# wenbowen123/iros20-6d-pose-tracking

Measured on AMD Instinct MI355X. Metric: RGB-D pair inferences/sec (176x176), higher is better.
Workload: dtype f32; 1 GPU; configs[1]: batch=64 synthetic 176x176 RGB-D pairs per GPU, random-init Se3TrackNet (reference state_dict surface), stage=full; pairs_per_gpu=64, global_batch=64, stage=full, frames=resident in HBM

## Files before the change

iros20-6d-pose-tracking_amd/csrc/wino64_fused.hip:

```cpp
#include "mfma_common.h"

namespace se3tn {

namespace {
constexpr int W64_TILES = 11;
constexpr int W64_PATCH = 2 * W64_TILES + 2;
constexpr int W64_PATCH_FLOATS = W64_PATCH * W64_PATCH * 32;
constexpr int W64_V_FLOATS = 128 * 32, W64_U_FLOATS = 64 * 32;
constexpr int W64_UBUFS = 2;
constexpr int W64_LDS_FLOATS = W64_PATCH_FLOATS + 2 * W64_V_FLOATS + W64_UBUFS * W64_U_FLOATS;
constexpr int W64_YLDS_FLOATS = W64_TILES * W64_TILES * (4 * 64 + 4);
constexpr size_t W64_LDS_BYTES = sizeof(float) * (W64_YLDS_FLOATS > W64_LDS_FLOATS ? W64_YLDS_FLOATS : W64_LDS_FLOATS);
}

__device__ __forceinline__ void bt_row(int i, int& r0, int& r1, float& c0, float& c1) {
  r0 = i == 0 ? 0 : 1;
  r1 = i == 3 ? 3 : 2;
  c0 = i == 2 ? -1.f : 1.f;
  c1 = (i == 0 || i == 3) ? -1.f : 1.f;
}
__device__ __forceinline__ void at_col(int i, float& a0, float& a1) {
  a0 = i == 3 ? 0.f : 1.f;
  a1 = i == 0 ? 0.f : (i == 1 ? 1.f : -1.f);
}

template <bool NA, bool NB>
__device__ __forceinline__ float add_pm(const float a, const float b) {
  float r;
  if constexpr (!NA && !NB) asm volatile("v_add_f32 %0, %1, %2" : "=v"(r) : "v"(a), "v"(b));
  else if constexpr (NA && !NB) asm volatile("v_sub_f32 %0, %2, %1" : "=v"(r) : "v"(a), "v"(b));
  else if constexpr (!NA && NB) asm volatile("v_sub_f32 %0, %1, %2" : "=v"(r) : "v"(a), "v"(b));
  else asm volatile("v_sub_f32 %0, -%1, %2" : "=v"(r) : "v"(a), "v"(b));
  return r;
}
template <int K>
__device__ __forceinline__ void acc_pm(float& y, const float m) {
  if constexpr (K > 0) asm volatile("v_add_f32 %0, %0, %1" : "+v"(y) : "v"(m));
  else if constexpr (K < 0) asm volatile("v_sub_f32 %0, %0, %1" : "+v"(y) : "v"(m));
}
struct W64Tab {
  static constexpr int bt_r0(int i) { return i == 0 ? 0 : 1; }
  static constexpr int bt_r1(int i) { return i == 3 ? 3 : 2; }
  static constexpr bool bt_n0(int i) { return i == 2; }
  static constexpr bool bt_n1(int i) { return i == 0 || i == 3; }
  static constexpr int at(int y, int i) { return y == 0 ? (i == 3 ? 0 : 1) : (i == 0 ? 0 : (i == 1 ? 1 : -1)); }
  static constexpr int off(int r, int s) { return (r * W64_PATCH + (s >> 1) + 12 * (s & 1)) * 32; }
};

struct Wino64Args {
  const float* in;
  const float* U;
  const float* bias;
  const float* res;
  float* out;
  int in_ld, res_ld, out_ld;
  int in_gs, res_gs, out_gs, bias_gs;
  long long u_gs;
  int n, groups;
};

template <int EPI>
__global__ __launch_bounds__(512) void wino64_fused_kernel(const Wino64Args a) {
  extern __shared__ __attribute__((aligned(16))) float smem[];
  float* patch = smem;
  float* Vb = smem + W64_PATCH_FLOATS;
  float* Ub = Vb + 2 * W64_V_FLOATS;

  const int tid = threadIdx.x, lane = tid & 63;
  const int wid = __builtin_amdgcn_readfirstlane(tid >> 6);
  const int rb = wid >> 1, cbk = wid & 1;
  const int l31 = lane & 31, hh = lane >> 5;

  const int g = blockIdx.x % a.groups, rest = blockIdx.x / a.groups;
  const int quad = rest & 3, img = rest >> 2;
  const int y0 = (quad >> 1) * 2 * W64_TILES, x0 = (quad & 1) * 2 * W64_TILES;
  constexpr int HP = 46;
  const float* __restrict__ in = a.in + (size_t)g * a.in_gs + ((size_t)(img * HP + y0) * HP + x0) * a.in_ld;
  const float* __restrict__ Ug = a.U + (size_t)g * a.u_gs;
  const unsigned lds0 = __builtin_amdgcn_readfirstlane(lds_addr_of(smem));

  const int ur = tid >> 3;
  const unsigned uvoff = (unsigned)(lds_rows::stage_src(ur, tid & 7) * 4);

#define W64_ISSUE_PATCH(CH)                                                                                     \
  {                                                                                                            \
    const float* pb_ = in + (CH) * 32;                                                                          \
    _Pragma("unroll") for (int j_ = 0; j_ < 9; ++j_) {                                \
      const int id_ = tid + 512 * j_, px_ = id_ >> 3, py_ = px_ / W64_PATCH, pxx_ = px_ - py_ * W64_PATCH;      \
      const int xs_ = pxx_ < 12 ? 2 * pxx_ : 2 * pxx_ - 23;           \
      glds16<0>(pb_, (unsigned)(((py_ * HP + xs_) * a.in_ld + (id_ & 7) * 4) * 4),                              \
                lds0 + (unsigned)((wid * 64 + 512 * j_) * 16));                                                 \
    }                                                                                                          \
  }
#define W64_ISSUE_U(CH, F, BUFI)                                                                                \
  glds16<0>(Ug + (size_t)((CH) * 16 + (F)) * W64_U_FLOATS, uvoff,                                              \
            lds0 + (unsigned)((W64_PATCH_FLOATS + 2 * W64_V_FLOATS + (BUFI) * W64_U_FLOATS + wid * 256) * 4));

  int tpix[2], tdst[2];
#pragma unroll
  for (int j = 0; j < 2; ++j) {
    const int tt = (tid + 512 * j) >> 3, tcb = tid & 7;
    const int ttr = tt < W64_TILES * W64_TILES ? tt : W64_TILES * W64_TILES - 1;
    const int tty = ttr / W64_TILES, ttx = ttr - tty * W64_TILES;
    tpix[j] = ((2 * tty) * W64_PATCH + ttx) * 32 + tcb * 4;
    tdst[j] = tt * 32 + lds_rows::slot_off(tt, tcb);
  }
#define W64_BT(F)                                                                                               \
  int r0_, r1_, s0_, s1_;                                                                                      \
  float cr0_, cr1_, cs0_, cs1_;                                                                                \
  bt_row((F) >> 2, r0_, r1_, cr0_, cr1_);                                                                      \
  bt_row((F) & 3, s0_, s1_, cs0_, cs1_);                                                                       \
  const int q0_ = (s0_ >> 1) + 12 * (s0_ & 1), q1_ = (s1_ >> 1) + 12 * (s1_ & 1);              \
  const int o00_ = (r0_ * W64_PATCH + q0_) * 32, o01_ = (r0_ * W64_PATCH + q1_) * 32;                          \
  const int o10_ = (r1_ * W64_PATCH + q0_) * 32, o11_ = (r1_ * W64_PATCH + q1_) * 32;                          \
  const float c00_ = cr0_ * cs0_, c01_ = cr0_ * cs1_, c10_ = cr1_ * cs0_, c11_ = cr1_ * cs1_;
#define W64_TR_LOAD(D)                                                                                          \
  _Pragma("unroll") for (int j_ = 0; j_ < 2; ++j_) {                                                            \
    D[j_][0] = *reinterpret_cast<const float4*>(patch + tpix[j_] + o00_);                                       \
    D[j_][1] = *reinterpret_cast<const float4*>(patch + tpix[j_] + o01_);                                       \
    D[j_][2] = *reinterpret_cast<const float4*>(patch + tpix[j_] + o10_);                                       \
    D[j_][3] = *reinterpret_cast<const float4*>(patch + tpix[j_] + o11_);                                       \
  }
#define W64_TR_STORE(D, VBUF)                                                                                   \
  _Pragma("unroll") for (int j_ = 0; j_ < 2; ++j_) {                                                            \
    float4 v_;                                                                                                 \
    v_.x = c00_ * D[j_][0].x + c01_ * D[j_][1].x + c10_ * D[j_][2].x + c11_ * D[j_][3].x;                       \
    v_.y = c00_ * D[j_][0].y + c01_ * D[j_][1].y + c10_ * D[j_][2].y + c11_ * D[j_][3].y;                       \
    v_.z = c00_ * D[j_][0].z + c01_ * D[j_][1].z + c10_ * D[j_][2].z + c11_ * D[j_][3].z;                       \
    v_.w = c00_ * D[j_][0].w + c01_ * D[j_][1].w + c10_ * D[j_][2].w + c11_ * D[j_][3].w;                       \
    *reinterpret_cast<float4*>(Vb + (VBUF) * W64_V_FLOATS + tdst[j_]) = v_;                                     \
  }
#define W64_TRANSFORM(F, VBUF)                                                                                  \
  {                                                                                                            \
    W64_BT(F)                                                                                                  \
    float4 d_[2][4];                                                                                           \
    W64_TR_LOAD(d_)                                                                                            \
    W64_TR_STORE(d_, VBUF)                                                                                     \
  }

  const lds_rows::LaneFrag fo = lds_rows::lane_frag(l31, hh);

  float Y[16][4];
#pragma unroll
  for (int e = 0; e < 16; ++e)
#pragma unroll
    for (int o = 0; o < 4; ++o) Y[e][o] = 0.f;

  W64_ISSUE_PATCH(0)
  W64_ISSUE_U(0, 0, 0)
  wait_dma_and_barrier();
  W64_TRANSFORM(0, 0)
  __syncthreads();

  f32x16 accA, accB;
#pragma unroll
  for (int e = 0; e < 16; ++e) accB[e] = 0.f;
  const f32x16 zero16 = {0.f, 0.f, 0.f, 0.f, 0.f, 0.f, 0.f, 0.f, 0.f, 0.f, 0.f, 0.f, 0.f, 0.f, 0.f, 0.f};
#define W64_FOLD(PREV, F)                                                                                       \
  {                                                                                                            \
    float ay0_, ay1_, ax0_, ax1_;                                                                              \
    at_col((F) >> 2, ay0_, ay1_);                                                                              \
    at_col((F) & 3, ax0_, ax1_);                                                                               \
    const float k00_ = ay0_ * ax0_, k01_ = ay0_ * ax1_, k10_ = ay1_ * ax0_, k11_ = ay1_ * ax1_;                \
    _Pragma("unroll") for (int e_ = 0; e_ < 16; ++e_) {                                                        \
      const float m_ = PREV[e_];                                                                               \
      Y[e_][0] += k00_ * m_; Y[e_][1] += k01_ * m_; Y[e_][2] += k10_ * m_; Y[e_][3] += k11_ * m_;              \
    }                                                                                                          \
  }
#define W64_MFMA(ACC)                                                                                        \
  ACC = q_ == 0 ? __builtin_amdgcn_mfma_f32_32x32x2f32(wv_[0], pv_[0], zero16, 0, 0, 0)                         \
                : __builtin_amdgcn_mfma_f32_32x32x2f32(wv_[q_], pv_[q_], ACC, 0, 0, 0);
#define W64_STEP(F, ACC, PREV)                                                                                  \
  {                                                                                                            \
    constexpr int f_ = (F), buf = f_ & 1, fn_ = (f_ + 1) & 15, fp_ = (f_ + 15) & 15;                            \
    const bool last_ = ch == 1 && f_ == 15;                                                                    \
    if (!last_) W64_ISSUE_U(f_ == 15 ? 1 : ch, fn_, buf ^ 1)                                                    \
    if (f_ == 15 && ch == 0) W64_ISSUE_PATCH(1)  \
    {                                                                                                          \
      const float* pP = Vb + buf * W64_V_FLOATS + (rb * 32 + l31) * 32;                                        \
      const float* pW = Ub + buf * W64_U_FLOATS + (cbk * 32 + l31) * 32;                                       \
      float pv_[16], wv_[16];                                                                                  \
      float d_[2][4][4], v_[2][4];                                       \
      *reinterpret_cast<float4*>(pv_ + 0) = *reinterpret_cast<const float4*>(pP + fo.o0);                         \
      *reinterpret_cast<float4*>(wv_ + 0) = *reinterpret_cast<const float4*>(pW + fo.o0);                         \
      *reinterpret_cast<float4*>(pv_ + 4) = *reinterpret_cast<const float4*>(pP + fo.o1);                         \
      *reinterpret_cast<float4*>(wv_ + 4) = *reinterpret_cast<const float4*>(pW + fo.o1);                         \
      *reinterpret_cast<float4*>(pv_ + 8) = *reinterpret_cast<const float4*>(pP + fo.o2);                         \
      *reinterpret_cast<float4*>(wv_ + 8) = *reinterpret_cast<const float4*>(pW + fo.o2);                         \
      *reinterpret_cast<float4*>(pv_ + 12) = *reinterpret_cast<const float4*>(pP + fo.o3);                        \
      *reinterpret_cast<float4*>(wv_ + 12) = *reinterpret_cast<const float4*>(pW + fo.o3);                        \
                              \
       \
      constexpr int i_ = fn_ >> 2, j_ = fn_ & 3;                                                               \
      constexpr int oo_[4] = {W64Tab::off(W64Tab::bt_r0(i_), W64Tab::bt_r0(j_)), W64Tab::off(W64Tab::bt_r0(i_), W64Tab::bt_r1(j_)), \
                              W64Tab::off(W64Tab::bt_r1(i_), W64Tab::bt_r0(j_)), W64Tab::off(W64Tab::bt_r1(i_), W64Tab::bt_r1(j_))}; \
      constexpr bool nn_[4] = {W64Tab::bt_n0(i_) != W64Tab::bt_n0(j_), W64Tab::bt_n0(i_) != W64Tab::bt_n1(j_),  \
                               W64Tab::bt_n1(i_) != W64Tab::bt_n0(j_), W64Tab::bt_n1(i_) != W64Tab::bt_n1(j_)}; \
      _Pragma("unroll") for (int t_ = 0; t_ < 2; ++t_)                                                          \
        _Pragma("unroll") for (int w_ = 0; w_ < 4; ++w_)                                                        \
          *reinterpret_cast<float4*>(d_[t_][w_]) = *reinterpret_cast<const float4*>(patch + tpix[t_] + oo_[w_]); \
      constexpr int pi_ = fp_ >> 2, pj_ = fp_ & 3;    \
      __builtin_amdgcn_sched_barrier(0);                                                                       \
      _Pragma("unroll") for (int q_ = 0; q_ < 16; ++q_) {                                                       \
        W64_MFMA(ACC)                                                                                          \
        __builtin_amdgcn_sched_barrier(0);                                                                     \
        if (q_ < 8) {                             \
          _Pragma("unroll") for (int e_ = 2 * q_; e_ < 2 * q_ + 2; ++e_) {                                      \
            const float m_ = PREV[e_];                                                                         \
            acc_pm<W64Tab::at(0, pi_) * W64Tab::at(0, pj_)>(Y[e_][0], m_);                                     \
            acc_pm<W64Tab::at(0, pi_) * W64Tab::at(1, pj_)>(Y[e_][1], m_);                                     \
            acc_pm<W64Tab::at(1, pi_) * W64Tab::at(0, pj_)>(Y[e_][2], m_);                                     \
            acc_pm<W64Tab::at(1, pi_) * W64Tab::at(1, pj_)>(Y[e_][3], m_);                                     \
          }                                                                                                    \
        } else {               \
          const int t_ = (q_ - 8) >> 2, x_ = (q_ - 8) & 3;                                                     \
          v_[t_][x_] = add_pm<false, false>(add_pm<nn_[0], nn_[1]>(d_[t_][0][x_], d_[t_][1][x_]),              \
                                            add_pm<nn_[2], nn_[3]>(d_[t_][2][x_], d_[t_][3][x_]));             \
        }                                                                                                      \
        __builtin_amdgcn_sched_barrier(0);                                                                     \
      }                                                                                                        \
      *reinterpret_cast<float4*>(Vb + (buf ^ 1) * W64_V_FLOATS + tdst[0]) = *reinterpret_cast<float4*>(v_[0]); \
      *reinterpret_cast<float4*>(Vb + (buf ^ 1) * W64_V_FLOATS + tdst[1]) = *reinterpret_cast<float4*>(v_[1]); \
    }                                                                                                          \
    if (!last_) wait_dma_and_barrier();                                                                        \
    if (f_ == 15 && ch == 0) {  \
      W64_TRANSFORM(0, 0)                                                                                      \
      __syncthreads();                                                                                         \
    }                                                                                                          \
  }
  for (int ch = 0; ch < 2; ++ch) {
    W64_STEP(0, accA, accB) W64_STEP(1, accB, accA) W64_STEP(2, accA, accB) W64_STEP(3, accB, accA)
    W64_STEP(4, accA, accB) W64_STEP(5, accB, accA) W64_STEP(6, accA, accB) W64_STEP(7, accB, accA)
    W64_STEP(8, accA, accB) W64_STEP(9, accB, accA) W64_STEP(10, accA, accB) W64_STEP(11, accB, accA)
    W64_STEP(12, accA, accB) W64_STEP(13, accB, accA) W64_STEP(14, accA, accB) W64_STEP(15, accB, accA)
  }
  W64_FOLD(accB, 15)
#undef W64_STEP
#undef W64_MFMA
#undef W64_FOLD
#undef W64_ISSUE_PATCH
#undef W64_ISSUE_U
#undef W64_TRANSFORM
#undef W64_TR_LOAD
#undef W64_TR_STORE
#undef W64_BT

  constexpr int YS = 4 * 64 + 4;
  __syncthreads();
  {
    const int t = rb * 32 + l31;
    if (t < W64_TILES * W64_TILES) {
#pragma unroll
      for (int o = 0; o < 4; ++o)
#pragma unroll
        for (int q = 0; q < 4; ++q)
          *reinterpret_cast<float4*>(smem + t * YS + o * 64 + cbk * 32 + q * 8 + hh * 4) =
              make_float4(Y[4 * q + 0][o], Y[4 * q + 1][o], Y[4 * q + 2][o], Y[4 * q + 3][o]);
    }
  }
  const float* __restrict__ bias = a.bias + (size_t)g * a.bias_gs;
  const float* __restrict__ res = (EPI == 1) ? a.res + (size_t)g * a.res_gs : nullptr;
  float* __restrict__ out = a.out + (size_t)g * a.out_gs;
  const int c4 = (tid & 15) * 4;
  __syncthreads();
  const float4 b = *reinterpret_cast<const float4*>(bias + c4);
#pragma unroll 4
  for (int k = 0; k < 16; ++k) {
    const int p = (k * 512 + tid) >> 4;
    const int t = p >> 2, o = p & 3;
    if (t < W64_TILES * W64_TILES) {
      const int ty = t / W64_TILES, tx = t - ty * W64_TILES;
      const int oy = y0 + 2 * ty + (o >> 1) + 1, ox = x0 + 2 * tx + (o & 1) + 1;
      const size_t pix = (size_t)(img * HP + oy) * HP + ox;
      float4 v = *reinterpret_cast<const float4*>(smem + t * YS + o * 64 + c4);
      v.x += b.x; v.y += b.y; v.z += b.z; v.w += b.w;
      if (EPI == 1) {
        const float4 r = *reinterpret_cast<const float4*>(res + pix * a.res_ld + c4);
        v.x += r.x; v.y += r.y; v.z += r.z; v.w += r.w;
      }
      v.x = fmaxf(v.x, 0.f); v.y = fmaxf(v.y, 0.f); v.z = fmaxf(v.z, 0.f); v.w = fmaxf(v.w, 0.f);
      *reinterpret_cast<float4*>(out + pix * a.out_ld + c4) = v;
    }
  }
}

hipError_t launch_wino64(const float* in, int in_ld, int in_gs, const float* U, long long u_gs, const float* bias, int bias_gs,
                         const float* res, int res_ld, int res_gs, float* out, int out_ld, int out_gs, int n, int groups, int epi,
                         hipStream_t st) {
  Wino64Args a{};
  a.in = in; a.U = U; a.bias = bias; a.res = res; a.out = out;
  a.in_ld = in_ld; a.res_ld = res_ld; a.out_ld = out_ld;
  a.in_gs = in_gs; a.res_gs = res_gs; a.out_gs = out_gs; a.bias_gs = bias_gs; a.u_gs = u_gs;
  a.n = n; a.groups = groups;
  static PerDeviceOnce attr[2];
  const size_t lds = W64_LDS_BYTES;
  hipError_t e = epi == 1 ? set_lds(wino64_fused_kernel<1>, lds, attr[1]) : set_lds(wino64_fused_kernel<0>, lds, attr[0]);
  if (e != hipSuccess) return e;
  const dim3 grid(n * 4 * groups);
  if (epi == 1) hipLaunchKernelGGL(wino64_fused_kernel<1>, grid, dim3(512), lds, st, a);
  else hipLaunchKernelGGL(wino64_fused_kernel<0>, grid, dim3(512), lds, st, a);
  return hipGetLastError();
}

}
```

Baseline: 41830 pairs/s.

## Restructure Winograd 64-channel kernel around 16x16 MFMA with register-resident V tiles

Reworks the fused Winograd F(2x2,3x3) kernel so each wave owns 16 tiles and computes all 64 output channels with 16x16x4 MFMAs. The input transform is now done directly into registers instead of going through a V buffer in LDS. Filter tiles are prefetched in groups of four with explicit vmcnt waits, which removes the per-frequency barrier. The patch layout in LDS gets an XOR swizzle to reduce bank conflicts. The cost is more register pressure and a more intricate hand-tuned wait and barrier schedule, which is easy to get subtly wrong.

```diff
diff --git a/iros20-6d-pose-tracking_amd/csrc/wino64_fused.hip b/iros20-6d-pose-tracking_amd/csrc/wino64_fused.hip
--- a/iros20-6d-pose-tracking_amd/csrc/wino64_fused.hip
+++ b/iros20-6d-pose-tracking_amd/csrc/wino64_fused.hip
@@ -6,22 +6,14 @@
 constexpr int W64_TILES = 11;
 constexpr int W64_PATCH = 2 * W64_TILES + 2;
 constexpr int W64_PATCH_FLOATS = W64_PATCH * W64_PATCH * 32;
-constexpr int W64_V_FLOATS = 128 * 32, W64_U_FLOATS = 64 * 32;
-constexpr int W64_UBUFS = 2;
-constexpr int W64_LDS_FLOATS = W64_PATCH_FLOATS + 2 * W64_V_FLOATS + W64_UBUFS * W64_U_FLOATS;
+constexpr int W64_U_FLOATS = 64 * 32;
+constexpr int W64_UGROUP = 4;
+constexpr int W64_LDS_FLOATS = W64_PATCH_FLOATS + 2 * W64_UGROUP * W64_U_FLOATS;
 constexpr int W64_YLDS_FLOATS = W64_TILES * W64_TILES * (4 * 64 + 4);
 constexpr size_t W64_LDS_BYTES = sizeof(float) * (W64_YLDS_FLOATS > W64_LDS_FLOATS ? W64_YLDS_FLOATS : W64_LDS_FLOATS);
-}
-
-__device__ __forceinline__ void bt_row(int i, int& r0, int& r1, float& c0, float& c1) {
-  r0 = i == 0 ? 0 : 1;
-  r1 = i == 3 ? 3 : 2;
-  c0 = i == 2 ? -1.f : 1.f;
-  c1 = (i == 0 || i == 3) ? -1.f : 1.f;
-}
-__device__ __forceinline__ void at_col(int i, float& a0, float& a1) {
-  a0 = i == 3 ? 0.f : 1.f;
-  a1 = i == 0 ? 0.f : (i == 1 ? 1.f : -1.f);
+static_assert(W64_LDS_BYTES <= 163840, "one workgroup per CU: 160 KB of LDS");
+constexpr int W64_ROW = W64_PATCH * 32;
+typedef float f32x4 __attribute__((ext_vector_type(4)));
 }
 
 template <bool NA, bool NB>
@@ -44,7 +36,6 @@
   static constexpr bool bt_n0(int i) { return i == 2; }
   static constexpr bool bt_n1(int i) { return i == 0 || i == 3; }
   static constexpr int at(int y, int i) { return y == 0 ? (i == 3 ? 0 : 1) : (i == 0 ? 0 : (i == 1 ? 1 : -1)); }
-  static constexpr int off(int r, int s) { return (r * W64_PATCH + (s >> 1) + 12 * (s & 1)) * 32; }
 };
 
 struct Wino64Args {
@@ -59,17 +50,14 @@
   int n, groups;
 };
 
+#define W64_WAIT_BARRIER(N) asm volatile("s_waitcnt vmcnt(" #N ") lgkmcnt(0)\n\ts_barrier" ::: "memory")
+
 template <int EPI>
 __global__ __launch_bounds__(512) void wino64_fused_kernel(const Wino64Args a) {
   extern __shared__ __attribute__((aligned(16))) float smem[];
-  float* patch = smem;
-  float* Vb = smem + W64_PATCH_FLOATS;
-  float* Ub = Vb + 2 * W64_V_FLOATS;
-
   const int tid = threadIdx.x, lane = tid & 63;
   const int wid = __builtin_amdgcn_readfirstlane(tid >> 6);
-  const int rb = wid >> 1, cbk = wid & 1;
-  const int l31 = lane & 31, hh = lane >> 5;
+  const int r16 = lane & 15, jq = lane >> 4;
 
   const int g = blockIdx.x % a.groups, rest = blockIdx.x / a.groups;
   const int quad = rest & 3, img = rest >> 2;
@@ -79,184 +67,156 @@
   const float* __restrict__ Ug = a.U + (size_t)g * a.u_gs;
   const unsigned lds0 = __builtin_amdgcn_readfirstlane(lds_addr_of(smem));
 
-  const int ur = tid >> 3;
-  const unsigned uvoff = (unsigned)(lds_rows::stage_src(ur, tid & 7) * 4);
-
 #define W64_ISSUE_PATCH(CH)                                                                                     \
   {                                                                                                            \
     const float* pb_ = in + (CH) * 32;                                                                          \
     _Pragma("unroll") for (int j_ = 0; j_ < 9; ++j_) {                                \
-      const int id_ = tid + 512 * j_, px_ = id_ >> 3, py_ = px_ / W64_PATCH, pxx_ = px_ - py_ * W64_PATCH;      \
-      const int xs_ = pxx_ < 12 ? 2 * pxx_ : 2 * pxx_ - 23;           \
-      glds16<0>(pb_, (unsigned)(((py_ * HP + xs_) * a.in_ld + (id_ & 7) * 4) * 4),                              \
+      const int id_ = tid + 512 * j_, px_ = id_ >> 3, py_ = px_ / W64_PATCH, lc_ = px_ - py_ * W64_PATCH;       \
+      const int xs_ = lc_ < 12 ? 2 * lc_ : 2 * lc_ - 23;                                                        \
+      glds16<0>(pb_, (unsigned)(((py_ * HP + xs_) * a.in_ld + (((id_ & 7) ^ (lc_ & 7)) << 2)) * 4),             \
                 lds0 + (unsigned)((wid * 64 + 512 * j_) * 16));                                                 \
     }                                                                                                          \
   }
-#define W64_ISSUE_U(CH, F, BUFI)                                                                                \
-  glds16<0>(Ug + (size_t)((CH) * 16 + (F)) * W64_U_FLOATS, uvoff,                                              \
-            lds0 + (unsigned)((W64_PATCH_FLOATS + 2 * W64_V_FLOATS + (BUFI) * W64_U_FLOATS + wid * 256) * 4));
-
-  int tpix[2], tdst[2];
-#pragma unroll
-  for (int j = 0; j < 2; ++j) {
-    const int tt = (tid + 512 * j) >> 3, tcb = tid & 7;
-    const int ttr = tt < W64_TILES * W64_TILES ? tt : W64_TILES * W64_TILES - 1;
-    const int tty = ttr / W64_TILES, ttx = ttr - tty * W64_TILES;
-    tpix[j] = ((2 * tty) * W64_PATCH + ttx) * 32 + tcb * 4;
-    tdst[j] = tt * 32 + lds_rows::slot_off(tt, tcb);
-  }
-#define W64_BT(F)                                                                                               \
-  int r0_, r1_, s0_, s1_;                                                                                      \
-  float cr0_, cr1_, cs0_, cs1_;                                                                                \
-  bt_row((F) >> 2, r0_, r1_, cr0_, cr1_);                                                                      \
-  bt_row((F) & 3, s0_, s1_, cs0_, cs1_);                                                                       \
-  const int q0_ = (s0_ >> 1) + 12 * (s0_ & 1), q1_ = (s1_ >> 1) + 12 * (s1_ & 1);              \
-  const int o00_ = (r0_ * W64_PATCH + q0_) * 32, o01_ = (r0_ * W64_PATCH + q1_) * 32;                          \
-  const int o10_ = (r1_ * W64_PATCH + q0_) * 32, o11_ = (r1_ * W64_PATCH + q1_) * 32;                          \
-  const float c00_ = cr0_ * cs0_, c01_ = cr0_ * cs1_, c10_ = cr1_ * cs0_, c11_ = cr1_ * cs1_;
-#define W64_TR_LOAD(D)                                                                                          \
-  _Pragma("unroll") for (int j_ = 0; j_ < 2; ++j_) {                                                            \
-    D[j_][0] = *reinterpret_cast<const float4*>(patch + tpix[j_] + o00_);                                       \
-    D[j_][1] = *reinterpret_cast<const float4*>(patch + tpix[j_] + o01_);                                       \
-    D[j_][2] = *reinterpret_cast<const float4*>(patch + tpix[j_] + o10_);                                       \
-    D[j_][3] = *reinterpret_cast<const float4*>(patch + tpix[j_] + o11_);                                       \
-  }
-#define W64_TR_STORE(D, VBUF)                                                                                   \
-  _Pragma("unroll") for (int j_ = 0; j_ < 2; ++j_) {                                                            \
-    float4 v_;                                                                                                 \
-    v_.x = c00_ * D[j_][0].x + c01_ * D[j_][1].x + c10_ * D[j_][2].x + c11_ * D[j_][3].x;                       \
-    v_.y = c00_ * D[j_][0].y + c01_ * D[j_][1].y + c10_ * D[j_][2].y + c11_ * D[j_][3].y;                       \
-    v_.z = c00_ * D[j_][0].z + c01_ * D[j_][1].z + c10_ * D[j_][2].z + c11_ * D[j_][3].z;                       \
-    v_.w = c00_ * D[j_][0].w + c01_ * D[j_][1].w + c10_ * D[j_][2].w + c11_ * D[j_][3].w;                       \
-    *reinterpret_cast<float4*>(Vb + (VBUF) * W64_V_FLOATS + tdst[j_]) = v_;                                     \
-  }
-#define W64_TRANSFORM(F, VBUF)                                                                                  \
+  const unsigned uvoff = (unsigned)(lds_rows::stage_src(tid >> 3, tid & 7) * 4);
+#define W64_ISSUE_U(T, P)                                                                                       \
+  glds16<0>(Ug + (size_t)(T) * W64_U_FLOATS, uvoff, lds0 + (unsigned)((W64_PATCH_FLOATS + (P) * W64_U_FLOATS + wid * 256) * 4));
+#define W64_ISSUE_UGROUP(T0, P0)                                                                                \
+  _Pragma("unroll") for (int k_ = 0; k_ < W64_UGROUP; ++k_) W64_ISSUE_U((T0) + k_, (P0) + k_)
+
+  const int tt = wid * 16 + r16;
+  const int ttr = tt < W64_TILES * W64_TILES ? tt : W64_TILES * W64_TILES - 1;
+  const int tty = ttr / W64_TILES, ttx = ttr - tty * W64_TILES;
+  int pb[4][2];
+#pragma unroll
+  for (int s = 0; s < 4; ++s) {
+    const int lc = (s & 1) ? 12 + ttx + (s >> 1) : ttx + (s >> 1);
+#pragma unroll
+    for (int h = 0; h < 2; ++h) pb[s][h] = ((2 * tty * W64_PATCH + lc) * 8 + ((jq + 4 * h) ^ (lc & 7))) * 4;
+  }
+  const float* up[2];
+#pragma unroll
+  for (int h = 0; h < 2; ++h) up[h] = smem + W64_PATCH_FLOATS + r16 * 32 + lds_rows::slot_off(r16, jq + 4 * h);
+#define W64_LOAD_U(DST, P)                                                                                      \
+  _Pragma("unroll") for (int b_ = 0; b_ < 4; ++b_) _Pragma("unroll") for (int h_ = 0; h_ < 2; ++h_)             \
+      DST[b_][h_] = *reinterpret_cast<const float4*>(up[h_] + (P) * W64_U_FLOATS + b_ * 512);
+#define W64_V0(VDST)                                                                                            \
+  _Pragma("unroll") for (int h_ = 0; h_ < 2; ++h_) {                                                            \
+    const float4 d00_ = *reinterpret_cast<const float4*>(smem + pb[0][h_]), d02_ = *reinterpret_cast<const float4*>(smem + pb[2][h_]); \
+    const float4 d20_ = *reinterpret_cast<const float4*>(smem + pb[0][h_] + 2 * W64_ROW);                       \
+    const float4 d22_ = *reinterpret_cast<const float4*>(smem + pb[2][h_] + 2 * W64_ROW);                       \
+    VDST[h_][0] = (d00_.x - d02_.x) - (d20_.x - d22_.x); VDST[h_][1] = (d00_.y - d02_.y) - (d20_.y - d22_.y);   \
+    VDST[h_][2] = (d00_.z - d02_.z) - (d20_.z - d22_.z); VDST[h_][3] = (d00_.w - d02_.w) - (d20_.w - d22_.w);   \
+  }
+
+  float Y[16][4];
+#pragma unroll
+  for (int e = 0; e < 16; ++e)
+#pragma unroll
+    for (int o = 0; o < 4; ++o) Y[e][o] = 0.f;
+
+  float4 Ua[4][2], Ub[4][2];
+  float Va[2][4], Vb[2][4];
+  f32x4 accA[4], accB[4];
+  const f32x4 zero4 = {0.f, 0.f, 0.f, 0.f};
+#pragma unroll
+  for (int b = 0; b < 4; ++b) accB[b] = zero4;
+
+  W64_ISSUE_PATCH(0)
+  W64_ISSUE_UGROUP(0, 0)
+  W64_ISSUE_UGROUP(4, 4)
+  W64_WAIT_BARRIER(4);
+  W64_LOAD_U(Ua, 0)
+  W64_V0(Va)
+
+#define W64_STEP(F, UC, UN, VC, VN, ACC, PREV)                                                                  \
   {                                                                                                            \
-    W64_BT(F)                                                                                                  \
-    float4 d_[2][4];                                                                                           \
-    W64_TR_LOAD(d_)                                                                                            \
-    W64_TR_STORE(d_, VBUF)                                                                                     \
-  }
-
-  const lds_rows::LaneFrag fo = lds_rows::lane_frag(l31, hh);
-
-  float Y[16][4];
-#pragma unroll
-  for (int e = 0; e < 16; ++e)
-#pragma unroll
-    for (int o = 0; o < 4; ++o) Y[e][o] = 0.f;
-
-  W64_ISSUE_PATCH(0)
-  W64_ISSUE_U(0, 0, 0)
-  wait_dma_and_barrier();
-  W64_TRANSFORM(0, 0)
-  __syncthreads();
-
-  f32x16 accA, accB;
-#pragma unroll
-  for (int e = 0; e < 16; ++e) accB[e] = 0.f;
-  const f32x16 zero16 = {0.f, 0.f, 0.f, 0.f, 0.f, 0.f, 0.f, 0.f, 0.f, 0.f, 0.f, 0.f, 0.f, 0.f, 0.f, 0.f};
-#define W64_FOLD(PREV, F)                                                                                       \
-  {                                                                                                            \
-    float ay0_, ay1_, ax0_, ax1_;                                                                              \
-    at_col((F) >> 2, ay0_, ay1_);                                                                              \
-    at_col((F) & 3, ax0_, ax1_);                                                                               \
-    const float k00_ = ay0_ * ax0_, k01_ = ay0_ * ax1_, k10_ = ay1_ * ax0_, k11_ = ay1_ * ax1_;                \
-    _Pragma("unroll") for (int e_ = 0; e_ < 16; ++e_) {                                                        \
-      const float m_ = PREV[e_];                                                                               \
-      Y[e_][0] += k00_ * m_; Y[e_][1] += k01_ * m_; Y[e_][2] += k10_ * m_; Y[e_][3] += k11_ * m_;              \
-    }                                                                                                          \
-  }
-#define W64_MFMA(ACC)                                                                                        \
-  ACC = q_ == 0 ? __builtin_amdgcn_mfma_f32_32x32x2f32(wv_[0], pv_[0], zero16, 0, 0, 0)                         \
-                : __builtin_amdgcn_mfma_f32_32x32x2f32(wv_[q_], pv_[q_], ACC, 0, 0, 0);
-#define W64_STEP(F, ACC, PREV)                                                                                  \
-  {                                                                                                            \
-    constexpr int f_ = (F), buf = f_ & 1, fn_ = (f_ + 1) & 15, fp_ = (f_ + 15) & 15;                            \
-    const bool last_ = ch == 1 && f_ == 15;                                                                    \
-    if (!last_) W64_ISSUE_U(f_ == 15 ? 1 : ch, fn_, buf ^ 1)                                                    \
-    if (f_ == 15 && ch == 0) W64_ISSUE_PATCH(1)  \
-    {                                                                                                          \
-      const float* pP = Vb + buf * W64_V_FLOATS + (rb * 32 + l31) * 32;                                        \
-      const float* pW = Ub + buf * W64_U_FLOATS + (cbk * 32 + l31) * 32;                                       \
-      float pv_[16], wv_[16];                                                                                  \
-      float d_[2][4][4], v_[2][4];                                       \
-      *reinterpret_cast<float4*>(pv_ + 0) = *reinterpret_cast<const float4*>(pP + fo.o0);                         \
-      *reinterpret_cast<float4*>(wv_ + 0) = *reinterpret_cast<const float4*>(pW + fo.o0);                         \
-      *reinterpret_cast<float4*>(pv_ + 4) = *reinterpret_cast<const float4*>(pP + fo.o1);                         \
-      *reinterpret_cast<float4*>(wv_ + 4) = *reinterpret_cast<const float4*>(pW + fo.o1);                         \
-      *reinterpret_cast<float4*>(pv_ + 8) = *reinterpret_cast<const float4*>(pP + fo.o2);                         \
-      *reinterpret_cast<float4*>(wv_ + 8) = *reinterpret_cast<const float4*>(pW + fo.o2);                         \
-      *reinterpret_cast<float4*>(pv_ + 12) = *reinterpret_cast<const float4*>(pP + fo.o3);                        \
-      *reinterpret_cast<float4*>(wv_ + 12) = *reinterpret_cast<const float4*>(pW + fo.o3);                        \
-                              \
-       \
-      constexpr int i_ = fn_ >> 2, j_ = fn_ & 3;                                                               \
-      constexpr int oo_[4] = {W64Tab::off(W64Tab::bt_r0(i_), W64Tab::bt_r0(j_)), W64Tab::off(W64Tab::bt_r0(i_), W64Tab::bt_r1(j_)), \
-                              W64Tab::off(W64Tab::bt_r1(i_), W64Tab::bt_r0(j_)), W64Tab::off(W64Tab::bt_r1(i_), W64Tab::bt_r1(j_))}; \
-      constexpr bool nn_[4] = {W64Tab::bt_n0(i_) != W64Tab::bt_n0(j_), W64Tab::bt_n0(i_) != W64Tab::bt_n1(j_),  \
-                               W64Tab::bt_n1(i_) != W64Tab::bt_n0(j_), W64Tab::bt_n1(i_) != W64Tab::bt_n1(j_)}; \
-      _Pragma("unroll") for (int t_ = 0; t_ < 2; ++t_)                                                          \
-        _Pragma("unroll") for (int w_ = 0; w_ < 4; ++w_)                                                        \
-          *reinterpret_cast<float4*>(d_[t_][w_]) = *reinterpret_cast<const float4*>(patch + tpix[t_] + oo_[w_]); \
-      constexpr int pi_ = fp_ >> 2, pj_ = fp_ & 3;    \
+    constexpr int f_ = (F), fn_ = (f_ + 1) & 15, fp_ = (f_ + 15) & 15;                                          \
+    if ((f_ & 3) == 3) {                                                                                       \
+      if (f_ == 15 && ch == 0) W64_WAIT_BARRIER(9); else W64_WAIT_BARRIER(0);                                   \
+      constexpr int pn_ = ((f_ >> 2) & 1) * W64_UGROUP;           \
+      if (ch == 0 || f_ < 8) { W64_ISSUE_UGROUP(ch * 16 + f_ + 5, pn_) }                                        \
+    }                                                                                                          \
+    W64_LOAD_U(UN, ((fn_ >> 2) & 1) * W64_UGROUP + (fn_ & 3))    \
+    constexpr int i_ = fn_ >> 2, j_ = fn_ & 3;                                                                 \
+    constexpr int ra_ = W64Tab::bt_r0(i_) * W64_ROW, rb_ = W64Tab::bt_r1(i_) * W64_ROW;                         \
+    constexpr int sa_ = W64Tab::bt_r0(j_), sb_ = W64Tab::bt_r1(j_);                                            \
+    constexpr bool nn_[4] = {W64Tab::bt_n0(i_) != W64Tab::bt_n0(j_), W64Tab::bt_n0(i_) != W64Tab::bt_n1(j_),    \
+                             W64Tab::bt_n1(i_) != W64Tab::bt_n0(j_), W64Tab::bt_n1(i_) != W64Tab::bt_n1(j_)};   \
+    float d_[2][4][4];                                                                                         \
+    if (f_ != 15) {                                                                                            \
+      _Pragma("unroll") for (int h_ = 0; h_ < 2; ++h_) {                                                        \
+        *reinterpret_cast<float4*>(d_[h_][0]) = *reinterpret_cast<const float4*>(smem + pb[sa_][h_] + ra_);     \
+        *reinterpret_cast<float4*>(d_[h_][1]) = *reinterpret_cast<const float4*>(smem + pb[sb_][h_] + ra_);     \
+        *reinterpret_cast<float4*>(d_[h_][2]) = *reinterpret_cast<const float4*>(smem + pb[sa_][h_] + rb_);     \
+        *reinterpret_cast<float4*>(d_[h_][3]) = *reinterpret_cast<const float4*>(smem + pb[sb_][h_] + rb_);     \
+      }                                                                                                        \
+    }                                                                                                          \
+    if (f_ == 14 && ch == 0) {    \
+      asm volatile("s_waitcnt lgkmcnt(0)\n\ts_barrier" ::: "memory");                                           \
+      W64_ISSUE_PATCH(1)                                                                                       \
+    }                                                                                                          \
+    constexpr int pi_ = fp_ >> 2, pj_ = fp_ & 3;                                                               \
+    __builtin_amdgcn_sched_barrier(0);                                                                         \
+    _Pragma("unroll") for (int m_ = 0; m_ < 32; ++m_) {                                                         \
+      const int q_ = m_ >> 2, b_ = m_ & 3, h_ = q_ >> 2, k_ = q_ & 3;                                          \
+      const float ua_ = k_ == 0 ? UC[b_][h_].x : k_ == 1 ? UC[b_][h_].y : k_ == 2 ? UC[b_][h_].z : UC[b_][h_].w; \
+      ACC[b_] = q_ == 0 ? __builtin_amdgcn_mfma_f32_16x16x4f32(ua_, VC[h_][k_], zero4, 0, 0, 0)                 \
+                        : __builtin_amdgcn_mfma_f32_16x16x4f32(ua_, VC[h_][k_], ACC[b_], 0, 0, 0);              \
       __builtin_amdgcn_sched_barrier(0);                                                                       \
-      _Pragma("unroll") for (int q_ = 0; q_ < 16; ++q_) {                                                       \
-        W64_MFMA(ACC)                                                                                          \
-        __builtin_amdgcn_sched_barrier(0);                                                                     \
-        if (q_ < 8) {                             \
-          _Pragma("unroll") for (int e_ = 2 * q_; e_ < 2 * q_ + 2; ++e_) {                                      \
-            const float m_ = PREV[e_];                                                                         \
-            acc_pm<W64Tab::at(0, pi_) * W64Tab::at(0, pj_)>(Y[e_][0], m_);                                     \
-            acc_pm<W64Tab::at(0, pi_) * W64Tab::at(1, pj_)>(Y[e_][1], m_);                                     \
-            acc_pm<W64Tab::at(1, pi_) * W64Tab::at(0, pj_)>(Y[e_][2], m_);                                     \
-            acc_pm<W64Tab::at(1, pi_) * W64Tab::at(1, pj_)>(Y[e_][3], m_);                                     \
-          }                                                                                                    \
-        } else {               \
-          const int t_ = (q_ - 8) >> 2, x_ = (q_ - 8) & 3;                                                     \
-          v_[t_][x_] = add_pm<false, false>(add_pm<nn_[0], nn_[1]>(d_[t_][0][x_], d_[t_][1][x_]),              \
-                                            add_pm<nn_[2], nn_[3]>(d_[t_][2][x_], d_[t_][3][x_]));             \
-        }                                                                                                      \
-        __builtin_amdgcn_sched_barrier(0);                                                                     \
+      if (m_ < 16) {          \
+        const float m__ = PREV[m_ >> 2][m_ & 3];                                                                \
+        acc_pm<W64Tab::at(0, pi_) * W64Tab::at(0, pj_)>(Y[m_][0], m__);                                        \
+        acc_pm<W64Tab::at(0, pi_) * W64Tab::at(1, pj_)>(Y[m_][1], m__);                                        \
+        acc_pm<W64Tab::at(1, pi_) * W64Tab::at(0, pj_)>(Y[m_][2], m__);                                        \
+        acc_pm<W64Tab::at(1, pi_) * W64Tab::at(1, pj_)>(Y[m_][3], m__);                                        \
+      } else if (m_ < 24 && f_ != 15) {    \
+        const int t_ = (m_ - 16) >> 2, x_ = (m_ - 16) & 3;                                                     \
+        VN[t_][x_] = add_pm<false, false>(add_pm<nn_[0], nn_[1]>(d_[t_][0][x_], d_[t_][1][x_]),                \
+                                          add_pm<nn_[2], nn_[3]>(d_[t_][2][x_], d_[t_][3][x_]));               \
       }                                                                                                        \
-      *reinterpret_cast<float4*>(Vb + (buf ^ 1) * W64_V_FLOATS + tdst[0]) = *reinterpret_cast<float4*>(v_[0]); \
-      *reinterpret_cast<float4*>(Vb + (buf ^ 1) * W64_V_FLOATS + tdst[1]) = *reinterpret_cast<float4*>(v_[1]); \
-    }                                                                                                          \
-    if (!last_) wait_dma_and_barrier();                                                                        \
-    if (f_ == 15 && ch == 0) {  \
-      W64_TRANSFORM(0, 0)                                                                                      \
-      __syncthreads();                                                                                         \
+      __builtin_amdgcn_sched_barrier(0);                                                                       \
+    }                                                                                                          \
+    if (f_ == 15 && ch == 0) {    \
+      W64_WAIT_BARRIER(4);                                                                                     \
+      W64_V0(VN)                                                                                               \
     }                                                                                                          \
   }
   for (int ch = 0; ch < 2; ++ch) {
-    W64_STEP(0, accA, accB) W64_STEP(1, accB, accA) W64_STEP(2, accA, accB) W64_STEP(3, accB, accA)
-    W64_STEP(4, accA, accB) W64_STEP(5, accB, accA) W64_STEP(6, accA, accB) W64_STEP(7, accB, accA)
-    W64_STEP(8, accA, accB) W64_STEP(9, accB, accA) W64_STEP(10, accA, accB) W64_STEP(11, accB, accA)
-    W64_STEP(12, accA, accB) W64_STEP(13, accB, accA) W64_STEP(14, accA, accB) W64_STEP(15, accB, accA)
-  }
-  W64_FOLD(accB, 15)
+    W64_STEP(0, Ua, Ub, Va, Vb, accA, accB) W64_STEP(1, Ub, Ua, Vb, Va, accB, accA)
+    W64_STEP(2, Ua, Ub, Va, Vb, accA, accB) W64_STEP(3, Ub, Ua, Vb, Va, accB, accA)
+    W64_STEP(4, Ua, Ub, Va, Vb, accA, accB) W64_STEP(5, Ub, Ua, Vb, Va, accB, accA)
+    W64_STEP(6, Ua, Ub, Va, Vb, accA, accB) W64_STEP(7, Ub, Ua, Vb, Va, accB, accA)
+    W64_STEP(8, Ua, Ub, Va, Vb, accA, accB) W64_STEP(9, Ub, Ua, Vb, Va, accB, accA)
+    W64_STEP(10, Ua, Ub, Va, Vb, accA, accB) W64_STEP(11, Ub, Ua, Vb, Va, accB, accA)
+    W64_STEP(12, Ua, Ub, Va, Vb, accA, accB) W64_STEP(13, Ub, Ua, Vb, Va, accB, accA)
+    W64_STEP(14, Ua, Ub, Va, Vb, accA, accB) W64_STEP(15, Ub, Ua, Vb, Va, accB, accA)
+  }
+  {
+#pragma unroll
+    for (int e = 0; e < 16; ++e) {
+      const float m = accB[e >> 2][e & 3];
+      acc_pm<W64Tab::at(0, 3) * W64Tab::at(0, 3)>(Y[e][0], m);
+      acc_pm<W64Tab::at(0, 3) * W64Tab::at(1, 3)>(Y[e][1], m);
+      acc_pm<W64Tab::at(1, 3) * W64Tab::at(0, 3)>(Y[e][2], m);
+      acc_pm<W64Tab::at(1, 3) * W64Tab::at(1, 3)>(Y[e][3], m);
+    }
+  }
 #undef W64_STEP
-#undef W64_MFMA
-#undef W64_FOLD
+#undef W64_V0
+#undef W64_LOAD_U
+#undef W64_ISSUE_UGROUP
+#undef W64_ISSUE_U
 #undef W64_ISSUE_PATCH
-#undef W64_ISSUE_U
-#undef W64_TRANSFORM
-#undef W64_TR_LOAD
-#undef W64_TR_STORE
-#undef W64_BT
 
   constexpr int YS = 4 * 64 + 4;
   __syncthreads();
-  {
-    const int t = rb * 32 + l31;
-    if (t < W64_TILES * W64_TILES) {
-#pragma unroll
-      for (int o = 0; o < 4; ++o)
-#pragma unroll
-        for (int q = 0; q < 4; ++q)
-          *reinterpret_cast<float4*>(smem + t * YS + o * 64 + cbk * 32 + q * 8 + hh * 4) =
-              make_float4(Y[4 * q + 0][o], Y[4 * q + 1][o], Y[4 * q + 2][o], Y[4 * q + 3][o]);
-    }
+  if (tt < W64_TILES * W64_TILES) {
+#pragma unroll
+    for (int o = 0; o < 4; ++o)
+#pragma unroll
+      for (int b = 0; b < 4; ++b)
+        *reinterpret_cast<float4*>(smem + tt * YS + o * 64 + b * 16 + jq * 4) =
+            make_float4(Y[4 * b + 0][o], Y[4 * b + 1][o], Y[4 * b + 2][o], Y[4 * b + 3][o]);
   }
   const float* __restrict__ bias = a.bias + (size_t)g * a.bias_gs;
   const float* __restrict__ res = (EPI == 1) ? a.res + (size_t)g * a.res_gs : nullptr;
@@ -283,6 +243,7 @@
     }
   }
 }
+#undef W64_WAIT_BARRIER
 
 hipError_t launch_wino64(const float* in, int in_ld, int in_gs, const float* U, long long u_gs, const float* bias, int bias_gs,
                          const float* res, int res_ld, int res_gs, float* out, int out_ld, int out_gs, int n, int groups, int epi,
```

Result: no change. 42160 pairs/s (median of 6 runs) (+0.8%).
